# ysbbin/Robust-Object-Detection

Measured on NVIDIA B200. Metric: corrupted images/sec (1360x765 RGB), motion blur k=9, higher is better.
Workload: dtype u8

## Files before the change

robust-object-detection_b200/csrc/blur.cu:

```cuda

#include "rod_internal.h"

namespace rod {

struct BlurParams {
    const DevImage* images;
    const Tile* tiles;
    int n_tiles;
    const uint8_t* src;
    uint8_t* dst;
    const uint8_t* opcodes;
    int k;
    int row_buf_bytes;
    unsigned int* counter;
};

constexpr int kBlurLeft = 64;

__device__ __forceinline__ void cp_async16(uint32_t smem_addr, const void* gptr) {
    asm volatile("cp.async.cg.shared.global [%0], [%1], 16;" ::"r"(smem_addr), "l"(gptr) : "memory");
}
__device__ __forceinline__ void cp_async_wait_all() {
    asm volatile("cp.async.commit_group;\ncp.async.wait_group 0;" ::: "memory");
}
__device__ __forceinline__ void stg16_blur(void* p, uint4 v) {
    asm volatile("st.global.L1::no_allocate.v4.u32 [%0], {%1,%2,%3,%4};" ::"l"(p), "r"(v.x), "r"(v.y), "r"(v.z),
                 "r"(v.w)
                 : "memory");
}

template <int K>
__global__ void __launch_bounds__(256, 4) blur_rows_kernel(BlurParams p) {
    extern __shared__ __align__(16) uint8_t smem[];
    const int warp = threadIdx.x >> 5, lane = threadIdx.x & 31;
    uint8_t* buf = smem + (size_t)warp * p.row_buf_bytes;
    const uint32_t buf_s = (uint32_t)__cvta_generic_to_shared(buf);
    const int k = (K == 0) ? p.k : K;
    const int halo = 3 * (k >> 1);

    for (int sub = 8, ti = 0;;) {
        if (sub >= 8) {
            if (lane == 0) ti = (int)atomicAdd(p.counter, 1u);
            ti = __shfl_sync(0xFFFFFFFFu, ti, 0);
            sub = 0;
        }
        if (ti >= p.n_tiles) break;
        const Tile t = p.tiles[ti];
        const int wr = sub++;
        if (p.opcodes != nullptr && p.opcodes[t.img] != ROD_OP_BLUR) { sub = 8; continue; }
        if (wr >= t.b) { sub = 8; continue; }
        const DevImage im = p.images[t.img];
        const int y = t.a + wr;
        const int n = 3 * im.w;
        const uint8_t* srow = p.src + im.src_off + (int64_t)y * im.src_pitch;
        uint8_t* drow = p.dst + im.dst_off + (int64_t)y * im.dst_pitch;
        const int shift = (int)((uintptr_t)drow & 15);
        uint8_t* row = buf + kBlurLeft + shift;
        const int jf0 = (shift != 0) ? 1 : 0;
        const int jf1 = (n + shift) >> 4;
        const bool right_edge = ((n + shift) & 15) != 0;

        if ((((uintptr_t)srow ^ (uintptr_t)drow) & 15) == 0) {
            const uint8_t* sal = srow - shift;
            for (int j = jf0 + lane; j < jf1; j += 32) cp_async16(buf_s + kBlurLeft + 16 * j, sal + 16 * j);
            const int i = (lane < 16) ? (lane - shift) : (16 * jf1 - shift + lane - 16);
            if (((lane < 16) ? (shift != 0) : right_edge) && i >= 0 && i < n) row[i] = srow[i];
            cp_async_wait_all();
        } else {
            for (int i = lane; i < n; i += 32) row[i] = srow[i];
        }
        __syncwarp();
        if (lane < 2 * halo || K == 0) {
            for (int q = lane; q < 2 * halo; q += 32) {
                const int i = (q < halo) ? (q - halo) : (n + q - halo);
                const int px = (i >= 0) ? i / 3 : -((-i + 2) / 3);
                const int c = i - 3 * px;
                int rp;
                if (im.w > (k >> 1)) rp = (px < 0) ? -px : 2 * (im.w - 1) - px;
                else rp = reflect101(px, im.w);
                row[i] = row[3 * rp + c];
            }
        }
        __syncwarp();
        uint8_t* dal = drow - shift;
        if (K == 9) {
            for (int j = jf0 + lane; j < jf1; j += 32) {
                const uint4* wp = reinterpret_cast<const uint4*>(buf + kBlurLeft + 16 * j - 16);
                const uint4 a = wp[0], b = wp[1], c = wp[2];
                const uint32_t w[12] = {a.x, a.y, a.z, a.w, b.x, b.y, b.z, b.w, c.x, c.y, c.z, c.w};
                uint32_t out[4];
                blur9_chunk16(w, out);
                stg16_blur(dal + 16 * j, make_uint4(out[0], out[1], out[2], out[3]));
            }
            if (lane < 2 && ((lane == 0) ? (shift != 0) : right_edge)) {
                const int j = (lane == 0) ? 0 : jf1;
                const uint4* wp = reinterpret_cast<const uint4*>(buf + kBlurLeft + 16 * j - 16);
                const uint4 a = wp[0], b = wp[1], c = wp[2];
                const uint32_t w[12] = {a.x, a.y, a.z, a.w, b.x, b.y, b.z, b.w, c.x, c.y, c.z, c.w};
                uint32_t out[4];
                blur9_chunk16(w, out);
                const int lo = 16 * j - shift;
                for (int bb = 0; bb < 16; ++bb) {
                    const int i = lo + bb;
                    if (i >= 0 && i < n) drow[i] = (uint8_t)(out[bb >> 2] >> (8 * (bb & 3)));
                }
            }
        } else {
            const int nchunks = (shift + n + 15) >> 4;
            for (int j = lane; j < nchunks; j += 32) {
                const int lo = 16 * j - shift;
                uint32_t out[4];
#pragma unroll
                for (int g = 0; g < 4; ++g) {
                    uint32_t o = 0;
#pragma unroll
                    for (int b = 0; b < 4; ++b) {
                        const int i = lo + 4 * g + b;
                        const uint32_t v = (i >= 0 && i < n) ? blur_byte_generic(row, i, k) : 0u;
                        o |= v << (8 * b);
                    }
                    out[g] = o;
                }
                if (lo >= 0 && lo + 16 <= n) {
                    stg16_blur(dal + 16 * j, make_uint4(out[0], out[1], out[2], out[3]));
                } else {
                    for (int b = 0; b < 16; ++b) {
                        const int i = lo + b;
                        if (i >= 0 && i < n) drow[i] = (uint8_t)(out[b >> 2] >> (8 * (b & 3)));
                    }
                }
            }
        }
        __syncwarp();
    }
}

int launch_blur(const rod_plan* plan, const uint8_t* src, uint8_t* dst, int k, const uint8_t* opcodes,
                cudaStream_t stream, int img_lo, int img_hi) {
    const auto [tiles, n_tiles] = plan->blur_tiles.range(img_lo, img_hi);
    if (n_tiles == 0) return ROD_OK;
    BlurParams p;
    p.images = plan->d_images;
    p.tiles = tiles;
    p.n_tiles = n_tiles;
    p.src = src; p.dst = dst; p.opcodes = opcodes; p.k = k;
    const int row_bytes = 3 * plan->max_w;
    p.row_buf_bytes = kBlurLeft + ((15 + row_bytes + 15) & ~15) + 64;
    int warps = kBlurRowsPerTile;
    while (warps > 1 && (size_t)p.row_buf_bytes * warps > 227 * 1024) --warps;
    const size_t smem = (size_t)p.row_buf_bytes * warps;
    if (smem > 227 * 1024) return ROD_ERR_UNSUPPORTED;
    int ctas_per_sm = (int)((227 * 1024) / (smem + 1024));
    if (ctas_per_sm < 1) ctas_per_sm = 1;
    if (ctas_per_sm > 4) ctas_per_sm = 4;
    p.counter = plan->d_counters + (plan->launch_seq.fetch_add(1u) & (kCounterRing - 1u));
    ROD_CUDA(cudaMemsetAsync(p.counter, 0, sizeof(unsigned int), stream));
    const int grid = grid_for(plan, (p.n_tiles + warps - 1) / warps, ctas_per_sm);
    if (k == 9) {
        ROD_CUDA(cudaFuncSetAttribute(blur_rows_kernel<9>, cudaFuncAttributeMaxDynamicSharedMemorySize, (int)smem));
        blur_rows_kernel<9><<<grid, 32 * warps, smem, stream>>>(p);
    } else {
        ROD_CUDA(cudaFuncSetAttribute(blur_rows_kernel<0>, cudaFuncAttributeMaxDynamicSharedMemorySize, (int)smem));
        blur_rows_kernel<0><<<grid, 32 * warps, smem, stream>>>(p);
    }
    ROD_CUDA(cudaGetLastError());
    return ROD_OK;
}

}
```

robust-object-detection_b200/csrc/rod_core.h:

```cpp
#pragma once
#include <math.h>
#include <stdint.h>
#include <string.h>

#if defined(__CUDACC__)
#define ROD_HD __host__ __device__ __forceinline__
#else
#define ROD_HD inline
#endif

namespace rod {

struct DevImage {
    uint64_t src_off, dst_off;
    int64_t src_pitch, dst_pitch;
    uint64_t elem_base;
    int32_t h, w;
    int32_t shape_id;
    int32_t contiguous;
};

struct Tile {
    int32_t img, a, b, c;
};

enum AreaMode { AREA_GENERAL = 0, AREA_FAST2 = 1, AREA_FASTN = 2, AREA_IDENTITY = 3 };

struct DevShape {
    int32_t h, w, nh, nw;
    int32_t area_mode;
    int32_t ix, iy;
    int32_t xt, yt;
    uint32_t ax_first, ax_alpha;
    uint32_t ay_first, ay_alpha;
    uint32_t ax_count, ay_count;
    uint32_t lx_s0, lx_a;
    uint32_t ly_s, ly_b;
    float inv_area;
    int32_t lin_identity;
    int32_t x2;
    int32_t strip_rows;
    int32_t strip_half_rows;
    uint32_t ay_pack;
    int32_t ay_packed;
    uint32_t ly_rc;
    int32_t x2w;
    int32_t x2p;
    uint32_t ly_rc2;
    uint32_t ly_rc3;
    int32_t x2g;
    uint32_t hy_pack;
    int32_t x2h;
    int32_t x2i;
};

#if defined(__CUDA_ARCH__)
ROD_HD float fmul(float a, float b) { return __fmul_rn(a, b); }
ROD_HD float fadd(float a, float b) { return __fadd_rn(a, b); }
ROD_HD float frint(float a) { return rintf(a); }
ROD_HD float fadd_rz(float a, float b) { return __fadd_rz(a, b); }
ROD_HD uint32_t fbits(float a) { return __float_as_uint(a); }
ROD_HD float bitsf(uint32_t a) { return __uint_as_float(a); }
#else
ROD_HD float fmul(float a, float b) { volatile float r = a * b; return r; }
ROD_HD float fadd(float a, float b) { volatile float r = a + b; return r; }
ROD_HD float frint(float a) { return nearbyintf(a); }
ROD_HD float fadd_rz(float a, float b) { return (float)floor((double)a + (double)b); }
ROD_HD uint32_t fbits(float a) { uint32_t u; memcpy(&u, &a, 4); return u; }
ROD_HD float bitsf(uint32_t a) { float f; memcpy(&f, &a, 4); return f; }
#endif

ROD_HD int reflect101(int i, int n) {
    if (n == 1) return 0;
    int period = 2 * (n - 1);
    int m = i % period;
    if (m < 0) m += period;
    return m < n ? m : period - m;
}

ROD_HD uint32_t noise_px(float vf, float nz) {
    float s = fadd(vf, nz);
    s = fmaxf(s, 0.0f);
    s = fminf(s, 255.0f);
    return fbits(fadd_rz(s, 8388608.0f)) & 0xFFu;
}

ROD_HD uint32_t mulhi32(uint32_t a, uint32_t b) {
#if defined(__CUDA_ARCH__)
    return __umulhi(a, b);
#else
    return (uint32_t)(((uint64_t)a * (uint64_t)b) >> 32);
#endif
}

ROD_HD void philox4x32_10(uint32_t c0, uint32_t c1, uint32_t c2, uint32_t c3, uint32_t k0, uint32_t k1,
                          uint32_t r[4]) {
#pragma unroll
    for (int i = 0; i < 10; ++i) {
        uint32_t hi0 = mulhi32(0xD2511F53u, c0), lo0 = 0xD2511F53u * c0;
        uint32_t hi1 = mulhi32(0xCD9E8D57u, c2), lo1 = 0xCD9E8D57u * c2;
        uint32_t n0 = hi1 ^ c1 ^ k0;
        uint32_t n2 = hi0 ^ c3 ^ k1;
        c0 = n0; c1 = lo1; c2 = n2; c3 = lo0;
        k0 += 0x9E3779B9u; k1 += 0xBB67AE85u;
    }
    r[0] = c0; r[1] = c1; r[2] = c2; r[3] = c3;
}

struct PhiloxKeys {
    uint32_t rk[20];
};
inline PhiloxKeys philox_round_keys(uint32_t k0, uint32_t k1) {
    PhiloxKeys ks;
    for (int i = 0; i < 10; ++i) {
        ks.rk[2 * i] = k0 + (uint32_t)i * 0x9E3779B9u;
        ks.rk[2 * i + 1] = k1 + (uint32_t)i * 0xBB67AE85u;
    }
    return ks;
}
template <int ROUNDS>
ROD_HD void philox4x32_rk(uint32_t c0, uint32_t c1, uint32_t c2, uint32_t c3, const PhiloxKeys& ks, uint32_t r[4]) {
#if defined(__CUDA_ARCH__)
#pragma unroll
#endif
    for (int i = 0; i < ROUNDS; ++i) {
        uint32_t hi0 = mulhi32(0xD2511F53u, c0), lo0 = 0xD2511F53u * c0;
        uint32_t hi1 = mulhi32(0xCD9E8D57u, c2), lo1 = 0xCD9E8D57u * c2;
        uint32_t n0 = hi1 ^ c1 ^ ks.rk[2 * i];
        uint32_t n2 = hi0 ^ c3 ^ ks.rk[2 * i + 1];
        c0 = n0; c1 = lo1; c2 = n2; c3 = lo0;
    }
    r[0] = c0; r[1] = c1; r[2] = c2; r[3] = c3;
}
ROD_HD void philox4x32_10_rk(uint32_t c0, uint32_t c1, uint32_t c2, uint32_t c3, const PhiloxKeys& ks, uint32_t r[4]) {
    philox4x32_rk<10>(c0, c1, c2, c3, ks, r);
}

#define ROD_PHILOX_TAIL_FLIP 0x80000000u
#define ROD_NOISE_K_PER_SIGMA 1.17741002251547466f
#define ROD_ANGLE_SCALE 9.58737992428525768e-05f
#define ROD_ANGLE_BIAS (-804.247680664062500f)
ROD_HD bool philox_needs_tail(const uint32_t r[4]) {
    uint32_t m = r[0] < r[1] ? r[0] : r[1];
    const uint32_t m2 = r[2] < r[3] ? r[2] : r[3];
    m = m < m2 ? m : m2;
    return m < 0x10000u;
}
ROD_HD void gauss2(uint32_t rw, bool use_tail, uint32_t tw, float* s0, float* s1) {
#if defined(__CUDA_ARCH__)
    const float xh = bitsf(__byte_perm(rw, 0x4B000000u, 0x7432));
    const float xl = bitsf(__byte_perm(rw, 0x4B000000u, 0x7410));
    float u = fmaf(xh, 1.52587890625e-05f, -127.99999237060546875f);
    if (use_tail && rw < 0x10000u) u = fmaf((float)tw, 3.5527136788005009e-15f, 1.7763568394002505e-15f);
    float l2, rad;
    asm("lg2.approx.ftz.f32 %0, %1;" : "=f"(l2) : "f"(u));
    asm("sqrt.approx.ftz.f32 %0, %1;" : "=f"(rad) : "f"(-l2));
    const float th = fmaf(xl, ROD_ANGLE_SCALE, ROD_ANGLE_BIAS);
    *s0 = rad * __cosf(th);
    *s1 = rad * __sinf(th);
#else
    double u = ((double)(rw >> 16) + 0.5) * 1.52587890625e-05;
    if (use_tail && rw < 0x10000u) u = ((double)tw + 0.5) * 3.5527136788005009e-15;
    const double rad = sqrt(-log2(u));
    const double th = (8388608.0 + (double)(rw & 0xFFFFu)) * (double)ROD_ANGLE_SCALE + (double)ROD_ANGLE_BIAS;
    *s0 = (float)(rad * cos(th));
    *s1 = (float)(rad * sin(th));
#endif
}
ROD_HD void gauss8(const uint32_t r[4], const uint32_t* t, float s[8]) {
#if defined(__CUDA_ARCH__)
#pragma unroll
#endif
    for (int p = 0; p < 4; ++p) gauss2(r[p], t != nullptr, t != nullptr ? t[p] : 0u, &s[2 * p], &s[2 * p + 1]);
}
ROD_HD uint32_t noise_floor16(float s, float K) {
#if defined(__CUDA_ARCH__)
    return fbits(__fmaf_rd(s, K, 12582912.0f));
#else
    return (uint32_t)(int32_t)floor((double)s * (double)K) & 0xFFFFu;
#endif
}
#if defined(__CUDACC__)
__device__ __forceinline__ uint32_t philox_word(uint32_t word, const float* s, float K) {
    const uint32_t f01 = __byte_perm(noise_floor16(s[0], K), noise_floor16(s[1], K), 0x5410);
    const uint32_t f23 = __byte_perm(noise_floor16(s[2], K), noise_floor16(s[3], K), 0x5410);
    const uint32_t v01 = __byte_perm(word, 0u, 0x4140), v23 = __byte_perm(word, 0u, 0x4342);
    const uint32_t q01 = __viaddmin_s16x2_relu(f01, v01, 0x00FF00FFu);
    const uint32_t q23 = __viaddmin_s16x2_relu(f23, v23, 0x00FF00FFu);
    return __byte_perm(q01, q23, 0x6420);
}
#endif
ROD_HD uint32_t noise_philox_px(uint32_t v, float s, float K) {
    int x = (int)v + (int)(int16_t)(noise_floor16(s, K) & 0xFFFFu);
    return (uint32_t)(x < 0 ? 0 : (x > 255 ? 255 : x));
}

#define ROD_GAUSS_TABLE_MAX_SIGMA 20.0f
#define ROD_GAUSS_TABLE_MIN_SIGMA 3.0f
#define ROD_GAUSS_H4_STRETCH_A (-1.4657745851475e-3)
#define ROD_GAUSS_H4_STRETCH_B (2.4950155916569e-5)
#ifndef ROD_GAUSS_AUTO
#define ROD_GAUSS_AUTO 0
#define ROD_GAUSS_BOXMULLER 1
#define ROD_GAUSS_TABLE_PHILOX7 2
#endif
ROD_HD uint32_t h4_form_same(int32_t x) { return (uint32_t)x * 0x00010001u; }
ROD_HD uint32_t h4_form_diff(int32_t x) { return (uint32_t)x * 0xFFFF0001u; }
ROD_HD void h4_combine(uint32_t A, uint32_t B, uint32_t C, uint32_t D, uint32_t* e01, uint32_t* e23) {
    const uint32_t u = A + B + 0x80008000u, v = C + D;
    *e01 = u + v;
    *e23 = u - v;
}
ROD_HD int h4_word_k(uint32_t w, const int32_t* X, int j) {
    uint32_t e01, e23;
    h4_combine(h4_form_same(X[w & 0xFFu]), h4_form_diff(X[(w >> 8) & 0xFFu]), h4_form_same(X[(w >> 16) & 0xFFu]),
               h4_form_diff(X[w >> 24]), &e01, &e23);
    const uint32_t e = (j & 2) ? e23 : e01;
    return (int)(((j & 1) ? (e >> 24) : (e >> 8)) & 0xFFu) - 128;
}
ROD_HD uint32_t noise_table_px(uint32_t v, int k) {
    const int x = (int)v + k;
    return (uint32_t)(x < 0 ? 0 : (x > 255 ? 255 : x));
}

inline double ndtri_double(double p) {
    if (p > 0.5) return -ndtri_double(1.0 - p);
    static const double a[] = {-3.969683028665376e+01, 2.209460984245205e+02, -2.759285104469687e+02,
                               1.383577518672690e+02, -3.066479806614716e+01, 2.506628277459239e+00};
    static const double b[] = {-5.447609879822406e+01, 1.615858368580409e+02, -1.556989798598866e+02,
                               6.680131188771972e+01, -1.328068155288572e+01};
    static const double c[] = {-7.784894002430293e-03, -3.223964580411365e-01, -2.400758277161838e+00,
                               -2.549732539343734e+00, 4.374664141464968e+00, 2.938163982698783e+00};
    static const double d[] = {7.784695709041462e-03, 3.224671290700398e-01, 2.445134137142996e+00,
                               3.754408661907416e+00};
    double x;
    if (p < 0.02425) {
        const double q = sqrt(-2.0 * log(p));
        x = (((((c[0] * q + c[1]) * q + c[2]) * q + c[3]) * q + c[4]) * q + c[5]) /
            ((((d[0] * q + d[1]) * q + d[2]) * q + d[3]) * q + 1.0);
    } else {
        const double q = p - 0.5, r = q * q;
        x = (((((a[0] * r + a[1]) * r + a[2]) * r + a[3]) * r + a[4]) * r + a[5]) * q /
            (((((b[0] * r + b[1]) * r + b[2]) * r + b[3]) * r + b[4]) * r + 1.0);
    }
    for (int it = 0; it < 3; ++it) {
        const double e = 0.5 * erfc(-x * 0.70710678118654752440) - p;
        const double u = e * 2.50662827463100050242 * exp(0.5 * x * x);
        x -= u / (1.0 + 0.5 * x * u);
    }
    return x;
}

ROD_HD uint32_t blur_byte_generic(const uint8_t* row, int i, int k) {
    int r = k >> 1;
    int s = 0;
    for (int j = -r; j <= r; ++j) s += row[i + 3 * j];
    return (uint32_t)((2 * s + k) / (2 * k));
}

ROD_HD uint32_t win_byte(const uint32_t* w, int p) { return (w[p >> 2] >> (8 * (p & 3))) & 0xFFu; }

ROD_HD void blur9_chunk16(const uint32_t* w, uint32_t out[4]) {
    uint32_t C[43];
#pragma unroll
    for (int t = 0; t < 43; ++t) {
        const int q = t + 1;
        if (t < 3) { C[t] = 0u; continue; }
#if defined(__CUDA_ARCH__)
        C[t] = __dp4a(w[q >> 2], 1u << (8 * (q & 3)), C[t - 3]);
#else
        C[t] = C[t - 3] + win_byte(w, q);
#endif
    }
    const float c9 = 0.111111164093017578125f;
    uint32_t qv[16];
#pragma unroll
    for (int n = 0; n < 16; ++n) {
        const uint32_t xs = C[n + 27] - C[n] + 0x4B000000u;
        qv[n] = fbits(fmaf(bitsf(xs), c9, 7456540.0f));
    }
#pragma unroll
    for (int g = 0; g < 4; ++g) {
#if defined(__CUDA_ARCH__)
        const uint32_t lo = __byte_perm(qv[4 * g], qv[4 * g + 1], 0x0040);
        const uint32_t hi = __byte_perm(qv[4 * g + 2], qv[4 * g + 3], 0x0040);
        out[g] = __byte_perm(lo, hi, 0x5410);
#else
        out[g] = (qv[4 * g] & 0xFFu) | ((qv[4 * g + 1] & 0xFFu) << 8) | ((qv[4 * g + 2] & 0xFFu) << 16) |
                 ((qv[4 * g + 3] & 0xFFu) << 24);
#endif
    }
}

ROD_HD uint32_t area_value(const uint8_t* src, int64_t pitch, const DevShape& sh, const uint32_t* tab, int dy,
                           int dx, int c) {
    if (sh.area_mode == AREA_FAST2) {
        const uint8_t* p = src + (int64_t)(2 * dy) * pitch + (2 * dx) * 3 + c;
        return ((uint32_t)p[0] + p[3] + p[pitch] + p[pitch + 3] + 2u) >> 2;
    }
    if (sh.area_mode == AREA_IDENTITY) {
        return src[(int64_t)dy * pitch + dx * 3 + c];
    }
    if (sh.area_mode == AREA_FASTN) {
        uint32_t s = 0;
        for (int yy = 0; yy < sh.iy; ++yy) {
            const uint8_t* p = src + (int64_t)(dy * sh.iy + yy) * pitch + (dx * sh.ix) * 3 + c;
            for (int xx = 0; xx < sh.ix; ++xx) s += p[3 * xx];
        }
        float r = frint(fmul((float)s, sh.inv_area));
        r = r < 0.f ? 0.f : (r > 255.f ? 255.f : r);
        return (uint32_t)(int)r;
    }
    const int32_t* xfirst = (const int32_t*)(tab + sh.ax_first);
    const int32_t* xcount = (const int32_t*)(tab + sh.ax_count);
    const float* xalpha = (const float*)(tab + sh.ax_alpha) + dx * sh.xt;
    const int32_t* yfirst = (const int32_t*)(tab + sh.ay_first);
    const int32_t* ycount = (const int32_t*)(tab + sh.ay_count);
    const float* yalpha = (const float*)(tab + sh.ay_alpha) + dy * sh.yt;
    int sx0 = xfirst[dx], nx = xcount[dx];
    int sy0 = yfirst[dy], ny = ycount[dy];
    float sum = 0.f;
    for (int ty = 0; ty < ny; ++ty) {
        const uint8_t* p = src + (int64_t)(sy0 + ty) * pitch + sx0 * 3 + c;
        float buf = 0.f;
        for (int tx = 0; tx < nx; ++tx) buf = fadd(buf, fmul((float)p[3 * tx], xalpha[tx]));
        float prod = fmul(yalpha[ty], buf);
        sum = (ty == 0) ? prod : fadd(sum, prod);
    }
    float r = frint(sum);
    r = r < 0.f ? 0.f : (r > 255.f ? 255.f : r);
    return (uint32_t)(int)r;
}

ROD_HD uint32_t funnel_r(uint32_t lo, uint32_t hi, int sh) {
#if defined(__CUDA_ARCH__)
    return __funnelshift_r(lo, hi, sh);
#else
    return (uint32_t)((((uint64_t)hi << 32) | lo) >> sh);
#endif
}
ROD_HD uint32_t sum_b0_b3(uint32_t w, uint32_t acc) {
#if defined(__CUDA_ARCH__)
    return __dp4a(w, 0x01000001u, acc);
#else
    return acc + (w & 0xFFu) + (w >> 24);
#endif
}
ROD_HD void pair_sums12(uint32_t w0, uint32_t w1, uint32_t w2, const uint32_t acc[6], uint32_t s[6]) {
    s[0] = sum_b0_b3(w0, acc[0]);
    s[1] = sum_b0_b3(funnel_r(w0, w1, 8), acc[1]);
    s[2] = sum_b0_b3(funnel_r(w0, w1, 16), acc[2]);
    s[3] = sum_b0_b3(funnel_r(w1, w2, 16), acc[3]);
    s[4] = sum_b0_b3(funnel_r(w1, w2, 24), acc[4]);
    s[5] = sum_b0_b3(w2, acc[5]);
}
ROD_HD void area_fast2_unit(const uint32_t r0[3], const uint32_t r1[3], uint32_t out6[6]) {
    const uint32_t two[6] = {2u, 2u, 2u, 2u, 2u, 2u};
    uint32_t s[6];
    pair_sums12(r0[0], r0[1], r0[2], two, s);
    pair_sums12(r1[0], r1[1], r1[2], s, s);
#pragma unroll
    for (int q = 0; q < 6; ++q) out6[q] = s[q] >> 2;
}
ROD_HD void area_x2f_accumulate(const uint32_t r[3], float beta, bool first, float acc[6]) {
    const uint32_t magic[6] = {0x4B000000u, 0x4B000000u, 0x4B000000u, 0x4B000000u, 0x4B000000u, 0x4B000000u};
    uint32_t s[6];
    pair_sums12(r[0], r[1], r[2], magic, s);
    const float nb = fmul(beta, -8388608.0f);
#pragma unroll
    for (int q = 0; q < 6; ++q) {
        const float prod = fmaf(bitsf(s[q]), beta, nb);
        acc[q] = first ? prod : fadd(acc[q], prod);
    }
}
ROD_HD void area_x2f_finish(const float acc[6], uint32_t out6[6]) {
#pragma unroll
    for (int q = 0; q < 6; ++q) out6[q] = fbits(fmaf(acc[q], 0.5f, 12582912.0f));
}

ROD_HD uint32_t linear_h4(uint32_t s0v, uint32_t s1v, uint32_t a_packed) {
    return (s0v * (a_packed & 0xFFFFu) + s1v * (a_packed >> 16)) >> 4;
}
ROD_HD uint32_t linear_v(uint32_t h0, uint32_t h1, uint32_t b_packed) {
    return ((((b_packed & 0xFFFFu) * h0) >> 16) + (((b_packed >> 16) * h1) >> 16) + 2u) >> 2;
}

ROD_HD uint32_t dot2_lo(uint32_t w16x2, uint32_t bytes, uint32_t acc) {
#if defined(__CUDA_ARCH__)
    return __dp2a_lo(w16x2, bytes, acc);
#else
    return acc + (w16x2 & 0xFFFFu) * (bytes & 0xFFu) + (w16x2 >> 16) * ((bytes >> 8) & 0xFFu);
#endif
}
ROD_HD uint32_t dot2_hi(uint32_t w16x2, uint32_t bytes, uint32_t acc) {
#if defined(__CUDA_ARCH__)
    return __dp2a_hi(w16x2, bytes, acc);
#else
    return acc + (w16x2 & 0xFFFFu) * ((bytes >> 16) & 0xFFu) + (w16x2 >> 16) * (bytes >> 24);
#endif
}
ROD_HD uint32_t x2_gather(const uint32_t* win, int a) {
#if defined(__CUDA_ARCH__)
    const int k = a >> 2, o = a & 3;
    return __byte_perm(win[k], win[k + 1], (o) | ((o + 3) << 4) | ((o + 1) << 8) | ((o + 4) << 12));
#else
    const uint8_t* b = (const uint8_t*)win;
    return (uint32_t)b[a] | ((uint32_t)b[a + 3] << 8) | ((uint32_t)b[a + 1] << 16) | ((uint32_t)b[a + 4] << 24);
#endif
}
ROD_HD void x2_expand24(const uint32_t win[5], float x[24]) {
    const uint32_t W31 = 6u | (2u << 16), W13 = 2u | (6u << 16), M = 0x4A800000u;
#pragma unroll
    for (int m = 0; m < 5; ++m) {
        const uint32_t g01 = x2_gather(win, 3 * m);
        const uint32_t g2x = x2_gather(win, 3 * m + 2);
        const int podd = 2 * m - 1, peven = 2 * m;
        if (podd >= 0) {
            x[3 * podd + 0] = bitsf(dot2_lo(W31, g01, M));
            x[3 * podd + 1] = bitsf(dot2_hi(W31, g01, M));
            x[3 * podd + 2] = bitsf(dot2_lo(W31, g2x, M));
        }
        if (peven < 8) {
            x[3 * peven + 0] = bitsf(dot2_lo(W13, g01, M));
            x[3 * peven + 1] = bitsf(dot2_hi(W13, g01, M));
            x[3 * peven + 2] = bitsf(dot2_lo(W13, g2x, M));
        }
    }
}

struct X2Row {
    float c0s, c1s;
    float k0;
    float k2;
};
ROD_HD X2Row x2_row_consts(uint32_t b_packed) {
    X2Row r;
    const float b0 = (float)(b_packed & 0xFFFFu), b1 = (float)(b_packed >> 16);
    r.c0s = b0 * 4.8828125e-4f;
    r.c1s = b1 * 4.8828125e-4f;
    r.k0 = 8388608.0f - b0 * 2048.0f;
    r.k2 = 6291456.5f - b1 * 512.0f;
    return r;
}
ROD_HD uint32_t x2_vertical(float x0, float x1, const X2Row& r) {
#if defined(__CUDA_ARCH__)
    const float y1 = __fmaf_rz(x0, r.c0s, r.k0);
    const float y2 = __fmaf_rz(x1, r.c1s, y1);
    return __float_as_uint(__fmaf_rz(y2, 0.25f, r.k2));
#else
    const double y1 = floor((double)x0 * r.c0s + r.k0);
    const double y2 = floor((double)x1 * r.c1s + y1);
    return fbits((float)floor(y2 * 0.25 + r.k2));
#endif
}

template <int I0, int I1>
ROD_HD uint32_t pk2(uint32_t w) {
#if defined(__CUDA_ARCH__)
    return __byte_perm(w, 0u, I0 | (4 << 4) | (I1 << 8) | (4 << 12));
#else
    return ((w >> (8 * I0)) & 0xFFu) | (((w >> (8 * I1)) & 0xFFu) << 16);
#endif
}
template <int SEL>
ROD_HD uint32_t perm(uint32_t a, uint32_t b) {
#if defined(__CUDA_ARCH__)
    return __byte_perm(a, b, SEL);
#else
    const uint64_t v = ((uint64_t)b << 32) | a;
    uint32_t r = 0;
    for (int i = 0; i < 4; ++i) r |= (uint32_t)((v >> (8 * ((SEL >> (4 * i)) & 7))) & 0xFFu) << (8 * i);
    return r;
#endif
}
ROD_HD void x2p_area(const uint32_t r0[6], const uint32_t r1[6], uint32_t b[6]) {
    const uint32_t two = 0x00020002u;
    b[0] = pk2<1, 2>(r0[0]) + pk2<0, 1>(r0[1]) + (pk2<1, 2>(r1[0]) + pk2<0, 1>(r1[1]) + two);
    b[1] = pk2<2, 3>(r0[1]) + pk2<1, 2>(r0[2]) + (pk2<2, 3>(r1[1]) + pk2<1, 2>(r1[2]) + two);
    b[2] = pk2<1, 2>(r0[3]) + pk2<0, 1>(r0[4]) + (pk2<1, 2>(r1[3]) + pk2<0, 1>(r1[4]) + two);
    b[3] = pk2<2, 3>(r0[4]) + pk2<1, 2>(r0[5]) + (pk2<2, 3>(r1[4]) + pk2<1, 2>(r1[5]) + two);
    b[4] = perm<0x5410>(sum_b0_b3(r1[0], sum_b0_b3(r0[0], 2u)), sum_b0_b3(r1[2], sum_b0_b3(r0[2], 2u)));
    b[5] = perm<0x5410>(sum_b0_b3(r1[3], sum_b0_b3(r0[3], 2u)), sum_b0_b3(r1[5], sum_b0_b3(r0[5], 2u)));
#if defined(__CUDA_ARCH__)
#pragma unroll
#endif
    for (int i = 0; i < 6; ++i) b[i] = (b[i] & 0x03FC03FCu) << 2;
}
ROD_HD void x2p_patch_two_pixel(uint32_t b[6]) {
    b[2] = perm<0x7632>(b[1], b[4]);
    b[5] = b[1];
}
ROD_HD uint32_t x2p_n10(const uint32_t b[6]) { return perm<0x5432>(b[5], b[3]); }
ROD_HD void x2p_build(const uint32_t b[6], uint32_t left_n9, uint32_t left_n10, uint32_t right_b4, uint32_t right_b0,
                      bool first, bool last, uint32_t A[12], uint32_t Bp[12]) {
    uint32_t N[12], F[12];
    N[0] = perm<0x5410>(b[4], b[0]);
    N[1] = perm<0x5432>(b[0], b[4]);
    N[2] = b[0];
    N[3] = b[1];
    N[4] = perm<0x5432>(b[4], b[1]);
    N[5] = perm<0x7632>(b[1], b[4]);
    N[6] = perm<0x5410>(b[5], b[2]);
    N[7] = perm<0x5432>(b[2], b[5]);
    N[8] = b[2];
    N[9] = b[3];
    N[10] = x2p_n10(b);
    N[11] = perm<0x7632>(b[3], b[5]);
    const uint32_t lc01 = first ? N[0] : left_n9;
    const uint32_t lc2 = first ? N[1] : left_n10;
    const uint32_t rc0 = last ? b[3] : right_b4;
    const uint32_t rc12 = last ? N[11] : right_b0;
    F[0] = lc01;
    F[1] = perm<0x5410>(lc2, b[1]);
    F[2] = N[5];
    F[3] = N[0];
    F[4] = perm<0x5432>(b[0], b[5]);
    F[5] = N[8];
    F[6] = N[3];
    F[7] = perm<0x5432>(b[4], b[3]);
    F[8] = N[11];
    F[9] = N[6];
    F[10] = perm<0x5432>(b[2], rc0);
    F[11] = rc12;
#if defined(__CUDA_ARCH__)
#pragma unroll
#endif
    for (int t = 0; t < 12; ++t) {
        const uint32_t q16 = N[t] * 3u + F[t];
        A[t] = q16 & 0xFFC0FFC0u;
        Bp[t] = (q16 * 3u + 0x00800080u) & 0xFFC0FFC0u;
    }
}
ROD_HD void x2p_emit(const uint32_t near_bp[12], const uint32_t far_a[12], uint32_t w[6]) {
#if defined(__CUDA_ARCH__)
#pragma unroll
#endif
    for (int g = 0; g < 6; ++g)
        w[g] = perm<0x7531>(near_bp[2 * g] + far_a[2 * g], near_bp[2 * g + 1] + far_a[2 * g + 1]);
}

ROD_HD uint32_t x2_vertical_cfix(uint32_t b_packed) { return (0u - (((b_packed >> 16) & 31u) << 17)) * 0x00010001u; }
ROD_HD uint32_t x2_vertical_pair(float x0a, float x1a, float x0b, float x1b, float c0s, float c1s, float k0p, uint32_t cfix) {
#if defined(__CUDA_ARCH__)
    const float ya = __fmaf_rz(x1a, c1s, __fmaf_rz(x0a, c0s, k0p));
    const float yb = __fmaf_rz(x1b, c1s, __fmaf_rz(x0b, c0s, k0p));
    return __byte_perm(__float_as_uint(ya), __float_as_uint(yb), 0x5410) * 64u + cfix;
#else
    const double ya = floor((double)x1a * c1s + floor((double)x0a * c0s + k0p));
    const double yb = floor((double)x1b * c1s + floor((double)x0b * c0s + k0p));
    return ((fbits((float)ya) & 0xFFFFu) | (fbits((float)yb) << 16)) * 64u + cfix;
#endif
}
ROD_HD void x2f_pairsums(const uint32_t rw[6], uint32_t s[12]) {
    const uint32_t magic[6] = {0x4B000000u, 0x4B000000u, 0x4B000000u, 0x4B000000u, 0x4B000000u, 0x4B000000u};
    pair_sums12(rw[0], rw[1], rw[2], magic, s);
    pair_sums12(rw[3], rw[4], rw[5], magic, s + 6);
}
ROD_HD void x2f_mac(const uint32_t s[12], float beta, bool first, float acc[12]) {
    const float nb = fmul(beta, -8388608.0f);
#if defined(__CUDA_ARCH__)
#pragma unroll
#endif
    for (int q = 0; q < 12; ++q) {
        const float prod = fmaf(bitsf(s[q]), beta, nb);
        acc[q] = first ? prod : fadd(acc[q], prod);
    }
}

ROD_HD float byte_magic(const uint32_t* w, int i) {
#if defined(__CUDA_ARCH__)
    return __uint_as_float(__byte_perm(w[i >> 2], 0x4B000000u, 0x7440 | (i & 3)));
#else
    return bitsf(0x4B000000u | ((w[i >> 2] >> (8 * (i & 3))) & 0xFFu));
#endif
}
ROD_HD void x2g_hrow(const uint32_t w[7], const float al[12], float hb[12]) {
    float x[27];
#if defined(__CUDA_ARCH__)
#pragma unroll
#endif
    for (int i = 0; i < 27; ++i) x[i] = byte_magic(w, i);
#if defined(__CUDA_ARCH__)
#pragma unroll
#endif
    for (int p = 0; p < 4; ++p) {
        const float n0 = fmul(al[3 * p], -8388608.0f), n1 = fmul(al[3 * p + 1], -8388608.0f), n2 = fmul(al[3 * p + 2], -8388608.0f);
#if defined(__CUDA_ARCH__)
#pragma unroll
#endif
        for (int c = 0; c < 3; ++c) {
            const float t0 = fmaf(x[6 * p + c], al[3 * p], n0);
            const float t1 = fmaf(x[6 * p + 3 + c], al[3 * p + 1], n1);
            const float t2 = fmaf(x[6 * p + 6 + c], al[3 * p + 2], n2);
            hb[3 * p + c] = fadd(fadd(t0, t1), t2);
        }
    }
}
ROD_HD void x2g_hrow_pre(const uint32_t w[7], const float al[12], const float nal[12], float hb[12]) {
    float x[27];
#if defined(__CUDA_ARCH__)
#pragma unroll
#endif
    for (int i = 0; i < 27; ++i) x[i] = byte_magic(w, i);
#if defined(__CUDA_ARCH__)
#pragma unroll
#endif
    for (int p = 0; p < 4; ++p) {
#if defined(__CUDA_ARCH__)
#pragma unroll
#endif
        for (int c = 0; c < 3; ++c) {
            const float t0 = fmaf(x[6 * p + c], al[3 * p], nal[3 * p]);
            const float t1 = fmaf(x[6 * p + 3 + c], al[3 * p + 1], nal[3 * p + 1]);
            const float t2 = fmaf(x[6 * p + 6 + c], al[3 * p + 2], nal[3 * p + 2]);
            hb[3 * p + c] = fadd(fadd(t0, t1), t2);
        }
    }
}
ROD_HD void x2g_vmac(const float hb[12], float beta, bool first, float acc[12]) {
#if defined(__CUDA_ARCH__)
#pragma unroll
#endif
    for (int q = 0; q < 12; ++q) {
        const float prod = fmul(beta, hb[q]);
        acc[q] = first ? prod : fadd(acc[q], prod);
    }
}
ROD_HD void x2g_round12(const float acc[12], uint32_t own[3]) {
    uint32_t b[12];
#if defined(__CUDA_ARCH__)
#pragma unroll
#endif
    for (int q = 0; q < 12; ++q) b[q] = fbits(fadd(acc[q], 12582912.0f));
#if defined(__CUDA_ARCH__)
#pragma unroll
#endif
    for (int k = 0; k < 3; ++k)
        own[k] = perm<0x5410>(perm<0x0040>(b[4 * k], b[4 * k + 1]), perm<0x0040>(b[4 * k + 2], b[4 * k + 3]));
}
ROD_HD void x2g_replicate(uint32_t own[3], int valid, uint32_t left_px) {
    if (valid >= 4) return;
    if (valid <= 1) {
        const uint32_t p = valid == 0 ? (left_px >> 8) : own[0];
        own[0] = perm<0x0210>(p, p);
        own[1] = perm<0x1021>(p, p);
        own[2] = perm<0x2102>(p, p);
    } else if (valid == 2) {
        const uint32_t o1 = own[1];
        own[1] = perm<0x4354>(own[0], o1);
        own[2] = perm<0x5435>(own[0], o1);
    } else {
        own[2] = perm<0x4324>(own[1], own[2]);
    }
}
ROD_HD void x2g_expand24(const uint32_t win[5], const uint32_t coef[8], uint32_t slip, float x[24]) {
    const uint32_t M = 0x4B000000u;
    uint32_t g01[5], g2x[5];
#if defined(__CUDA_ARCH__)
#pragma unroll
#endif
    for (int m = 0; m < 5; ++m) { g01[m] = x2_gather(win, 3 * m); g2x[m] = x2_gather(win, 3 * m + 2); }
#if defined(__CUDA_ARCH__)
#pragma unroll
#endif
    for (int px = 0; px < 8; ++px) {
        const int k = px >> 1;
        uint32_t a = g01[k], b = g2x[k];
        if (px & 1) {
            const bool sl = (slip >> k) & 1u;
            a = sl ? g01[k] : g01[k + 1];
            b = sl ? g2x[k] : g2x[k + 1];
        }
        const uint32_t h0 = dot2_lo(coef[px], a, M), h1 = dot2_hi(coef[px], a, M), h2 = dot2_lo(coef[px], b, M);
#if defined(__CUDA_ARCH__)
        x[3 * px + 0] = __fmaf_rz(bitsf(h0), 0.0625f, 7864320.0f);
        x[3 * px + 1] = __fmaf_rz(bitsf(h1), 0.0625f, 7864320.0f);
        x[3 * px + 2] = __fmaf_rz(bitsf(h2), 0.0625f, 7864320.0f);
#else
        x[3 * px + 0] = (float)(8388608.0 + (double)((h0 - M) >> 4));
        x[3 * px + 1] = (float)(8388608.0 + (double)((h1 - M) >> 4));
        x[3 * px + 2] = (float)(8388608.0 + (double)((h2 - M) >> 4));
#endif
    }
}
ROD_HD X2Row x2g_row_consts(uint32_t b_packed) {
    X2Row r;
    const float b0 = (float)(b_packed & 0xFFFFu), b1 = (float)(b_packed >> 16);
    r.c0s = b0 * 1.52587890625e-05f;
    r.c1s = b1 * 1.52587890625e-05f;
    r.k0 = 8388608.0f - b0 * 128.0f;
    r.k2 = 6291456.5f - b1 * 32.0f;
    return r;
}


}
```

Baseline: 948,300.

## Blur k=9 rows with per-lane sliding running sums and swizzled shared staging

Replaces the atomic work counter with a static grid-stride assignment of row slots. For k=9, each lane now processes a run of 8 consecutive 16-byte chunks, carrying the prefix-sum state between chunks so each chunk needs only one new shared-memory load instead of three. Results are written back into shared memory in place and then stored to global memory in a coalesced pass. The shared buffer gets an XOR swizzle to avoid bank conflicts from the strided per-lane access, at the cost of extra padding, more complex indexing, and losing dynamic load balancing.

```diff
diff --git a/robust-object-detection_b200/csrc/blur.cu b/robust-object-detection_b200/csrc/blur.cu
--- a/robust-object-detection_b200/csrc/blur.cu
+++ b/robust-object-detection_b200/csrc/blur.cu
@@ -12,10 +12,24 @@
     const uint8_t* opcodes;
     int k;
     int row_buf_bytes;
-    unsigned int* counter;
 };
 
-constexpr int kBlurLeft = 64;
+constexpr int kBlurLeft = 128;
+constexpr int kBlur9Run = 8;
+
+template <int K>
+__device__ __forceinline__ int blur_smem(int b) {
+    return (K == 9) ? (b ^ (((b >> 7) & 7) << 4)) : b;
+}
+__device__ __forceinline__ uint4 lds16(uint32_t a) {
+    uint4 v;
+    asm volatile("ld.shared.v4.u32 {%0,%1,%2,%3}, [%4];" : "=r"(v.x), "=r"(v.y), "=r"(v.z), "=r"(v.w) : "r"(a));
+    return v;
+}
+
+__device__ __forceinline__ void sts16(uint32_t a, uint4 v) {
+    asm volatile("st.shared.v4.u32 [%0], {%1,%2,%3,%4};" ::"r"(a), "r"(v.x), "r"(v.y), "r"(v.z), "r"(v.w) : "memory");
+}
 
 __device__ __forceinline__ void cp_async16(uint32_t smem_addr, const void* gptr) {
     asm volatile("cp.async.cg.shared.global [%0], [%1], 16;" ::"r"(smem_addr), "l"(gptr) : "memory");
@@ -33,41 +47,40 @@
 __global__ void __launch_bounds__(256, 4) blur_rows_kernel(BlurParams p) {
     extern __shared__ __align__(16) uint8_t smem[];
     const int warp = threadIdx.x >> 5, lane = threadIdx.x & 31;
-    uint8_t* buf = smem + (size_t)warp * p.row_buf_bytes;
-    const uint32_t buf_s = (uint32_t)__cvta_generic_to_shared(buf);
+    const uint32_t smem_s = (uint32_t)__cvta_generic_to_shared(smem);
+    const uint32_t pad = ((smem_s + 127u) & ~127u) - smem_s;
+    uint8_t* buf = smem + pad + (size_t)warp * p.row_buf_bytes;
+    const uint32_t buf_s = smem_s + pad + (uint32_t)(warp * p.row_buf_bytes);
     const int k = (K == 0) ? p.k : K;
     const int halo = 3 * (k >> 1);
 
-    for (int sub = 8, ti = 0;;) {
-        if (sub >= 8) {
-            if (lane == 0) ti = (int)atomicAdd(p.counter, 1u);
-            ti = __shfl_sync(0xFFFFFFFFu, ti, 0);
-            sub = 0;
-        }
-        if (ti >= p.n_tiles) break;
-        const Tile t = p.tiles[ti];
-        const int wr = sub++;
-        if (p.opcodes != nullptr && p.opcodes[t.img] != ROD_OP_BLUR) { sub = 8; continue; }
-        if (wr >= t.b) { sub = 8; continue; }
+    const int n_warps = gridDim.x * (blockDim.x >> 5);
+    const int n_slots = 8 * p.n_tiles;
+    for (int slot = blockIdx.x * (blockDim.x >> 5) + warp; slot < n_slots; slot += n_warps) {
+        const Tile t = p.tiles[slot >> 3];
+        const int wr = slot & 7;
+        if (wr >= t.b) continue;
+        if (p.opcodes != nullptr && p.opcodes[t.img] != ROD_OP_BLUR) continue;
         const DevImage im = p.images[t.img];
         const int y = t.a + wr;
         const int n = 3 * im.w;
         const uint8_t* srow = p.src + im.src_off + (int64_t)y * im.src_pitch;
         uint8_t* drow = p.dst + im.dst_off + (int64_t)y * im.dst_pitch;
         const int shift = (int)((uintptr_t)drow & 15);
-        uint8_t* row = buf + kBlurLeft + shift;
+        const int row0 = kBlurLeft + shift;
         const int jf0 = (shift != 0) ? 1 : 0;
         const int jf1 = (n + shift) >> 4;
         const bool right_edge = ((n + shift) & 15) != 0;
 
         if ((((uintptr_t)srow ^ (uintptr_t)drow) & 15) == 0) {
             const uint8_t* sal = srow - shift;
-            for (int j = jf0 + lane; j < jf1; j += 32) cp_async16(buf_s + kBlurLeft + 16 * j, sal + 16 * j);
+            for (int j = jf0 + lane; j < jf1; j += 32)
+                cp_async16(buf_s + blur_smem<K>(kBlurLeft + 16 * j), sal + 16 * j);
             const int i = (lane < 16) ? (lane - shift) : (16 * jf1 - shift + lane - 16);
-            if (((lane < 16) ? (shift != 0) : right_edge) && i >= 0 && i < n) row[i] = srow[i];
+            if (((lane < 16) ? (shift != 0) : right_edge) && i >= 0 && i < n) buf[blur_smem<K>(row0 + i)] = srow[i];
             cp_async_wait_all();
         } else {
-            for (int i = lane; i < n; i += 32) row[i] = srow[i];
+            for (int i = lane; i < n; i += 32) buf[blur_smem<K>(row0 + i)] = srow[i];
         }
         __syncwarp();
         if (lane < 2 * halo || K == 0) {
@@ -78,24 +91,17 @@
                 int rp;
                 if (im.w > (k >> 1)) rp = (px < 0) ? -px : 2 * (im.w - 1) - px;
                 else rp = reflect101(px, im.w);
-                row[i] = row[3 * rp + c];
+                buf[blur_smem<K>(row0 + i)] = buf[blur_smem<K>(row0 + 3 * rp + c)];
             }
         }
         __syncwarp();
         uint8_t* dal = drow - shift;
         if (K == 9) {
-            for (int j = jf0 + lane; j < jf1; j += 32) {
-                const uint4* wp = reinterpret_cast<const uint4*>(buf + kBlurLeft + 16 * j - 16);
-                const uint4 a = wp[0], b = wp[1], c = wp[2];
-                const uint32_t w[12] = {a.x, a.y, a.z, a.w, b.x, b.y, b.z, b.w, c.x, c.y, c.z, c.w};
-                uint32_t out[4];
-                blur9_chunk16(w, out);
-                stg16_blur(dal + 16 * j, make_uint4(out[0], out[1], out[2], out[3]));
-            }
+            auto chunk_s = [&](int j) { return buf_s + (uint32_t)blur_smem<K>(kBlurLeft + 16 * j); };
+            auto chunk = [&](int j) { return lds16(chunk_s(j)); };
             if (lane < 2 && ((lane == 0) ? (shift != 0) : right_edge)) {
                 const int j = (lane == 0) ? 0 : jf1;
-                const uint4* wp = reinterpret_cast<const uint4*>(buf + kBlurLeft + 16 * j - 16);
-                const uint4 a = wp[0], b = wp[1], c = wp[2];
+                const uint4 a = chunk(j - 1), b = chunk(j), c = chunk(j + 1);
                 const uint32_t w[12] = {a.x, a.y, a.z, a.w, b.x, b.y, b.z, b.w, c.x, c.y, c.z, c.w};
                 uint32_t out[4];
                 blur9_chunk16(w, out);
@@ -105,7 +111,33 @@
                     if (i >= 0 && i < n) drow[i] = (uint8_t)(out[bb >> 2] >> (8 * (bb & 3)));
                 }
             }
+            for (int jp = 0; jp < jf1; jp += 32 * kBlur9Run) {
+                const int j0 = min(jp + kBlur9Run * lane, jf1);
+                const int nr = jf1 - j0;
+                const uint32_t line = buf_s + blur_smem<K>(kBlurLeft + 16 * j0);
+                const uint4 a = chunk(j0 - 1);
+                uint4 b = lds16(line);
+                Blur9Run run;
+                blur9_run_start(run, a.y, a.z, a.w, b.x, b.y, b.z);
+                __syncwarp();
+#pragma unroll
+                for (int r = 0; r < kBlur9Run; ++r) {
+                    if (r >= nr) break;
+                    const uint32_t ca = (r + 1 < kBlur9Run) ? (line ^ (16u * (r + 1))) : chunk_s(j0 + r + 1);
+                    const uint4 c = lds16(ca);
+                    uint32_t out[4];
+                    blur9_run_step(run, b.w, c.x, c.y, c.z, out);
+                    const uint4 o = make_uint4(out[0], out[1], out[2], out[3]);
+                    if (r >= kBlur9Run - 2 && lane == 31) stg16_blur(dal + 16 * (int64_t)(j0 + r), o);
+                    else sts16(ca, o);
+                    b = c;
+                }
+                __syncwarp();
+                const int je = min(jp + 32 * kBlur9Run - 2, jf1);
+                for (int j = max(jp, jf0) + lane; j < je; j += 32) stg16_blur(dal + 16 * j, lds16(chunk_s(j + 1)));
+            }
         } else {
+            const uint8_t* row = buf + row0;
             const int nchunks = (shift + n + 15) >> 4;
             for (int j = lane; j < nchunks; j += 32) {
                 const int lo = 16 * j - shift;
@@ -145,16 +177,14 @@
     p.n_tiles = n_tiles;
     p.src = src; p.dst = dst; p.opcodes = opcodes; p.k = k;
     const int row_bytes = 3 * plan->max_w;
-    p.row_buf_bytes = kBlurLeft + ((15 + row_bytes + 15) & ~15) + 64;
+    p.row_buf_bytes = (kBlurLeft + ((15 + row_bytes + 15) & ~15) + 64 + 127) & ~127;
     int warps = kBlurRowsPerTile;
-    while (warps > 1 && (size_t)p.row_buf_bytes * warps > 227 * 1024) --warps;
-    const size_t smem = (size_t)p.row_buf_bytes * warps;
+    while (warps > 1 && (size_t)p.row_buf_bytes * warps + 128 > 227 * 1024) --warps;
+    const size_t smem = (size_t)p.row_buf_bytes * warps + 128;
     if (smem > 227 * 1024) return ROD_ERR_UNSUPPORTED;
     int ctas_per_sm = (int)((227 * 1024) / (smem + 1024));
     if (ctas_per_sm < 1) ctas_per_sm = 1;
     if (ctas_per_sm > 4) ctas_per_sm = 4;
-    p.counter = plan->d_counters + (plan->launch_seq.fetch_add(1u) & (kCounterRing - 1u));
-    ROD_CUDA(cudaMemsetAsync(p.counter, 0, sizeof(unsigned int), stream));
     const int grid = grid_for(plan, (p.n_tiles + warps - 1) / warps, ctas_per_sm);
     if (k == 9) {
         ROD_CUDA(cudaFuncSetAttribute(blur_rows_kernel<9>, cudaFuncAttributeMaxDynamicSharedMemorySize, (int)smem));
diff --git a/robust-object-detection_b200/csrc/rod_core.h b/robust-object-detection_b200/csrc/rod_core.h
--- a/robust-object-detection_b200/csrc/rod_core.h
+++ b/robust-object-detection_b200/csrc/rod_core.h
@@ -290,6 +290,61 @@
                  ((qv[4 * g + 3] & 0xFFu) << 24);
 #endif
     }
+}
+
+struct Blur9Run {
+    uint32_t C[27];
+};
+
+ROD_HD void blur9_run_start(Blur9Run& s, uint32_t w1, uint32_t w2, uint32_t w3, uint32_t w4, uint32_t w5,
+                            uint32_t w6) {
+    const uint32_t w[6] = {w1, w2, w3, w4, w5, w6};
+#pragma unroll
+    for (int t = 0; t < 27; ++t) {
+        const int q = t + 1;
+        if (t < 3) { s.C[t] = 0u; continue; }
+#if defined(__CUDA_ARCH__)
+        s.C[t] = __dp4a(w[(q >> 2) - 1], 1u << (8 * (q & 3)), s.C[t - 3]);
+#else
+        s.C[t] = s.C[t - 3] + win_byte(w, q - 4);
+#endif
+    }
+}
+
+ROD_HD void blur9_run_step(Blur9Run& s, uint32_t w7, uint32_t w8, uint32_t w9, uint32_t w10, uint32_t out[4]) {
+    const uint32_t w[4] = {w7, w8, w9, w10};
+    uint32_t C[43];
+#pragma unroll
+    for (int t = 0; t < 27; ++t) C[t] = s.C[t];
+#pragma unroll
+    for (int t = 27; t < 43; ++t) {
+        const int q = t + 1;
+#if defined(__CUDA_ARCH__)
+        C[t] = __dp4a(w[(q >> 2) - 7], 1u << (8 * (q & 3)), C[t - 3]);
+#else
+        C[t] = C[t - 3] + win_byte(w, q - 28);
+#endif
+    }
+    const float c9 = 0.111111164093017578125f;
+    uint32_t qv[16];
+#pragma unroll
+    for (int n = 0; n < 16; ++n) {
+        const uint32_t xs = C[n + 27] - C[n] + 0x4B000000u;
+        qv[n] = fbits(fmaf(bitsf(xs), c9, 7456540.0f));
+    }
+#pragma unroll
+    for (int g = 0; g < 4; ++g) {
+#if defined(__CUDA_ARCH__)
+        const uint32_t lo = __byte_perm(qv[4 * g], qv[4 * g + 1], 0x0040);
+        const uint32_t hi = __byte_perm(qv[4 * g + 2], qv[4 * g + 3], 0x0040);
+        out[g] = __byte_perm(lo, hi, 0x5410);
+#else
+        out[g] = (qv[4 * g] & 0xFFu) | ((qv[4 * g + 1] & 0xFFu) << 8) | ((qv[4 * g + 2] & 0xFFu) << 16) |
+                 ((qv[4 * g + 3] & 0xFFu) << 24);
+#endif
+    }
+#pragma unroll
+    for (int t = 0; t < 27; ++t) s.C[t] = C[t + 16];
 }
 
 ROD_HD uint32_t area_value(const uint8_t* src, int64_t pitch, const DevShape& sh, const uint32_t* tab, int dy,
```

New measurement: 966,100 (median of 6 runs). 1.02x the previous value.
